# autowarefoundation/autoware_vision_pilot

Measured on NVIDIA H100. Metric: camera frames/sec @1080p multi-task, higher is better.
Workload: dtype f16

## Files before the change

autoware_vision_pilot_b200/csrc/conv_gemm.cu:

```cuda
#include "common.cuh"
#include "conv_gemm.cuh"
#include "ops_internal.h"
#include <cstdio>
#include <cstring>
#include <algorithm>

namespace vpb {

static constexpr int kMma = 256;
static constexpr int kEpilogue = 128;
static constexpr int kThreads = kMma + kEpilogue + 32;
static constexpr int kParts = kEpilogue / 128;
static constexpr int kMaxStages = 8;
static constexpr int kATileBytes = 128 * 128;
static constexpr int kMaxDynSmem = 227 * 1024 - 4096;
__host__ __device__ constexpr int acc_pitch(int bn) { return bn + 4; }
__host__ __device__ constexpr size_t acc_bytes(int bn) { return static_cast<size_t>(128) * acc_pitch(bn) * 4; }

__device__ __forceinline__ void acc_ld16(uint32_t t, uint32_t (&r)[16]) {
  const uint32_t a = t << 2;
#pragma unroll
  for (int i = 0; i < 4; ++i)
    asm volatile("ld.shared.v4.b32 {%0, %1, %2, %3}, [%4];"
                 : "=r"(r[4 * i]), "=r"(r[4 * i + 1]), "=r"(r[4 * i + 2]), "=r"(r[4 * i + 3])
                 : "r"(a + 16u * i)
                 : "memory");
}

struct EpiPix {
  bool ok;
  bool zero;
  uint32_t ooff;
  uint32_t roff;
  uint32_t fpix;
  uint32_t img;
};

template <class E, int NC, bool TILEK>
__device__ __forceinline__ void epilogue_chunks(const ConvKParams& p, uint32_t t_row, int n0,
                                                const float* sbias, int part, const EpiPix& px) {
  const bool split = TILEK && p.split;
  const int nchunks = p.BN >> 4;
  typename E::T* out = reinterpret_cast<typename E::T*>(p.out);
  const typename E::T* res = reinterpret_cast<const typename E::T*>(p.res);
  typename E::T* out_lo = reinterpret_cast<typename E::T*>(p.out_lo);
  const typename E::T* res_lo = reinterpret_cast<const typename E::T*>(p.res_lo);
  for (int chunk0 = part; chunk0 < nchunks; chunk0 += kParts * NC) {
    uint32_t rr[NC][16];
#pragma unroll
    for (int c = 0; c < NC; ++c) acc_ld16(t_row + (chunk0 + kParts * c) * 16, rr[c]);
    float v[NC][16];
#pragma unroll
    for (int c = 0; c < NC; ++c) {
      const float4* sb4 = reinterpret_cast<const float4*>(sbias + (chunk0 + kParts * c) * 16);
#pragma unroll
      for (int i = 0; i < 4; ++i) {
        const float4 b4 = sb4[i];
        const float2 lo = fadd2(make_float2(__uint_as_float(rr[c][4 * i]), __uint_as_float(rr[c][4 * i + 1])), make_float2(b4.x, b4.y));
        const float2 hi = fadd2(make_float2(__uint_as_float(rr[c][4 * i + 2]), __uint_as_float(rr[c][4 * i + 3])), make_float2(b4.z, b4.w));
        v[c][4 * i] = lo.x; v[c][4 * i + 1] = lo.y; v[c][4 * i + 2] = hi.x; v[c][4 * i + 3] = hi.y;
      }
    }
    if (p.act == ACT_GELU) {
#pragma unroll
      for (int c = 0; c < NC; ++c)
#pragma unroll
        for (int i = 0; i < 8; ++i) {
          const float2 g = act_gelu2(make_float2(v[c][2 * i], v[c][2 * i + 1]));
          v[c][2 * i] = g.x; v[c][2 * i + 1] = g.y;
        }
    } else if (p.act == ACT_SILU) {
#pragma unroll
      for (int c = 0; c < NC; ++c)
#pragma unroll
        for (int i = 0; i < 16; ++i) v[c][i] = act_silu(v[c][i]);
    } else if (p.act == ACT_SIGMOID) {
#pragma unroll
      for (int c = 0; c < NC; ++c)
#pragma unroll
        for (int i = 0; i < 16; ++i) v[c][i] = (n0 + (chunk0 + kParts * c) * 16 + i < p.Cout) ? act_sigmoid(v[c][i]) : 0.f;
    }
    if (p.mode == VPB_EPI_FINAL) {
      if (px.ok && chunk0 == 0) {
        const uint32_t plane = static_cast<uint32_t>(p.H * p.W);
        float* of = p.out_f32 + px.img * static_cast<uint32_t>(p.Cout) * plane;
#pragma unroll
        for (int i = 0; i < 16; ++i)
          if (i < p.Cout) of[i * plane + px.fpix] = v[0][i];
        if (p.out_cls) {
          uint8_t cls = 0;
          if (p.final_kind == VPB_FINAL_ARGMAX) {
            float best = v[0][0];
#pragma unroll
            for (int i = 1; i < 16; ++i)
              if (i < p.Cout && v[0][i] > best) { best = v[0][i]; cls = static_cast<uint8_t>(i); }
          } else if (p.final_kind == VPB_FINAL_THRESH) {
            cls = v[0][0] > 0.f ? 1 : 0;
          } else if (p.final_kind == VPB_FINAL_EGOLANES) {
            cls = (v[0][2] > 0.f) ? 2 : (v[0][1] > 0.f) ? 1 : (v[0][0] > 0.f) ? 0 : 255;
          }
          p.out_cls[px.img * plane + px.fpix] = cls;
        }
      }
    } else if (px.ok) {
      if (p.mode == VPB_EPI_ADD || p.mode == VPB_EPI_MULADD) {
        uint4 rv[NC][2];
        bool rok[NC][2];
#pragma unroll
        for (int c = 0; c < NC; ++c) {
          const int n = n0 + (chunk0 + kParts * c) * 16;
          const typename E::T* rp = res + (px.roff + n);
#pragma unroll
          for (int j = 0; j < 2; ++j) {
            rok[c][j] = (n + 8 * j < p.ldr) && (n + 8 * j < p.nlim);
            rv[c][j] = rok[c][j] ? *reinterpret_cast<const uint4*>(rp + 8 * j) : make_uint4(0, 0, 0, 0);
          }
        }
        uint4 rl[NC][2];
#pragma unroll
        for (int c = 0; c < NC; ++c)
#pragma unroll
          for (int j = 0; j < 2; ++j)
            rl[c][j] = (split && rok[c][j])
                           ? *reinterpret_cast<const uint4*>(res_lo + (px.roff + n0 + (chunk0 + kParts * c) * 16) + 8 * j)
                           : make_uint4(0, 0, 0, 0);
#pragma unroll
        for (int c = 0; c < NC; ++c)
#pragma unroll
          for (int j = 0; j < 2; ++j) {
            if (!rok[c][j]) continue;
            const uint32_t rw[4] = {rv[c][j].x, rv[c][j].y, rv[c][j].z, rv[c][j].w};
            const uint32_t rwl[4] = {rl[c][j].x, rl[c][j].y, rl[c][j].z, rl[c][j].w};
#pragma unroll
            for (int i = 0; i < 4; ++i) {
              float2 f = unpack2<E>(rw[i]);
              if (split) { const float2 fl = unpack2<E>(rwl[i]); f.x += fl.x; f.y += fl.y; }
              float& a = v[c][8 * j + 2 * i];
              float& b = v[c][8 * j + 2 * i + 1];
              if (p.mode == VPB_EPI_ADD) { a += f.x; b += f.y; }
              else { a = fmaf(a, f.x, f.x); b = fmaf(b, f.y, f.y); }
              if (TILEK && p.act2 == ACT_SILU) { a = act_silu(a); b = act_silu(b); }
            }
          }
      }
#pragma unroll
      for (int c = 0; c < NC; ++c) {
        const int n = n0 + (chunk0 + kParts * c) * 16;
        typename E::T* op = out + (px.ooff + n);
#pragma unroll
        for (int j = 0; j < 2; ++j) {
          if (n + 8 * j < p.nlim) {
            uint4 o;
            o.x = pack2<E>(v[c][8 * j + 0], v[c][8 * j + 1]);
            o.y = pack2<E>(v[c][8 * j + 2], v[c][8 * j + 3]);
            o.z = pack2<E>(v[c][8 * j + 4], v[c][8 * j + 5]);
// ... 290 lines not shown
      if (et < BN) {
        const int nn = n0 + et;
        s_bias[et] = (p.bias && nn < p.Cout) ? __ldg(p.bias + (p.upc ? 4 * p.Cout : 0) + nn) : 0.f;
      }
      named_bar_sync(1, kEpilogue);
      mbar_wait_quiet(smem_u32(&acc_full), acc_phase);

      if (p.upc) {
        const int pa = ph >> 1, pb = ph & 1;
        const int cy = (pa == 0 && h == 0) ? 0 : (pa == 1 && h == p.H - 1) ? 2 : 1;
        const int cx = (pb == 0 && w == 0) ? 0 : (pb == 1 && w == p.W - 1) ? 2 : 1;
        const int cls = cy * 3 + cx;
        const float* gb = cls != 4 ? p.bias + cls * p.Cout + n0 : nullptr;
        const int oh = 2 * h + pa, ow = 2 * w + pb;
        EpiPix px;
        px.ok = (h < p.H) && (w < p.W);
        px.zero = false;
        px.ooff = img * p.out_img + static_cast<uint32_t>((oh + p.out_pad) * (Wo + 2 * p.out_pad) + (ow + p.out_pad)) * p.ldo;
        px.roff = 0; px.fpix = 0; px.img = 0;
        if (p.act == ACT_GELU) epilogue_store_fast<E, ACT_GELU, false, true>(p, t_row, n0, s_bias, part, px, gb);
        else epilogue_store_fast<E, ACT_NONE, false, true>(p, t_row, n0, s_bias, part, px, gb);
      } else {
        const int oh = (p.phases > 1) ? 2 * h + (ph >> 1) : h;
        const int ow = (p.phases > 1) ? 2 * w + (ph & 1) : w;
        EpiPix px;
        px.ok = (h < p.H) && (w < p.W);
        px.zero = false;
        px.ooff = img * p.out_img + static_cast<uint32_t>((oh + p.out_pad) * (Wo + 2 * p.out_pad) + (ow + p.out_pad)) * p.ldo;
        px.roff = img * p.res_img + static_cast<uint32_t>((oh + p.res_pad) * (Wo + 2 * p.res_pad) + (ow + p.res_pad)) * p.ldr;
        px.fpix = static_cast<uint32_t>(h * p.W + w);
        px.img = static_cast<uint32_t>(img);
        epilogue_tile<E>(p, t_row, n0, s_bias, part, px);
      }
      mbar_arrive(smem_u32(&acc_empty));
      acc_phase ^= 1u;
    }
  }
}

__global__ void zero_border_kernel(uint4* out, int H, int W, int ldo, int nlim) {
  pdl_wait();
  out += (static_cast<size_t>(blockIdx.y) * (H + 2) * (W + 2) * ldo) >> 3;
  const int per = nlim >> 3, nb = 2 * (W + 2) + 2 * H;
  for (int i = blockIdx.x * blockDim.x + threadIdx.x; i < nb * per; i += gridDim.x * blockDim.x) {
    const int pix = i / per, v = i - pix * per;
    int y, x;
    if (pix < W + 2) { y = 0; x = pix; }
    else if (pix < 2 * (W + 2)) { y = H + 1; x = pix - (W + 2); }
    else { const int q = pix - 2 * (W + 2); y = 1 + (q >> 1); x = (q & 1) ? W + 1 : 0; }
    out[((static_cast<size_t>(y) * (W + 2) + x) * ldo >> 3) + v] = make_uint4(0, 0, 0, 0);
  }
}



typedef CUresult (*EncodeTiledFn)(CUtensorMap*, CUtensorMapDataType, cuuint32_t, void*,
                                  const cuuint64_t*, const cuuint64_t*, const cuuint32_t*,
                                  const cuuint32_t*, CUtensorMapInterleave, CUtensorMapSwizzle,
                                  CUtensorMapL2promotion, CUtensorMapFloatOOBfill);

static EncodeTiledFn get_encode_fn() {
  static EncodeTiledFn fn = nullptr;
  if (!fn) {
    void* p = nullptr;
    cudaDriverEntryPointQueryResult q;
    if (cudaGetDriverEntryPoint("cuTensorMapEncodeTiled", &p, cudaEnableDefault, &q) ==
            cudaSuccess &&
        q == cudaDriverEntryPointSuccess)
      fn = reinterpret_cast<EncodeTiledFn>(p);
  }
  return fn;
}

int device_sm_count() {
  int dev = 0, n = 0;
  cudaGetDevice(&dev);
  cudaDeviceGetAttribute(&n, cudaDevAttrMultiProcessorCount, dev);
  return n > 0 ? n : 132;
}

static int pick_bn(int Cout, int want) {
  if (want > 0) return want <= 16 ? 16 : want <= 32 ? 32 : want <= 64 ? 64 : 128;
  for (int bn : {128, 64, 32}) {
    if (Cout <= bn && (Cout > bn / 2 || bn == 32)) return bn;
    if (Cout > bn && (Cout + bn - 1) / bn * bn - Cout <= Cout / 4) return bn;
  }
  return 16;
}

int conv_plan_build(const vpb_conv_args* a, ConvPlan* plan) {
  if (!a || !plan) return VPB_ERR_ARG;
  if (a->Cin <= 0 || (a->Cin & 7) || (a->ldi & 7) || a->ldi < a->Cin) {
    vpb_set_error("conv: Cin=%d ldi=%d must be multiples of 8 (ldi >= Cin)", a->Cin, a->ldi);
    return VPB_ERR_ARG;
  }
  const int cstride = a->stride == 2 ? 2 : 1;
  if (a->stride != 0 && a->stride != 1 && a->stride != 2) { vpb_set_error("conv: stride %d unsupported", a->stride); return VPB_ERR_ARG; }
  if (cstride == 2 && (a->algo == VPB_ALGO_LINEAR || a->phases != 1 || a->in_pad || a->in2 || a->in_lo)) {
    vpb_set_error("conv: stride 2 needs the TILE algorithm on an unpadded input, phases = 1, no second input");
    return VPB_ERR_ARG;
  }
  if (a->ldw != 0 && (a->ldw < a->Cin || (a->ldw & 7) || a->algo == VPB_ALGO_LINEAR)) {
    vpb_set_error("conv: ldw=%d must be a multiple of 8 >= Cin (TILE algorithm)", a->ldw);
    return VPB_ERR_ARG;
  }
  if (a->act2 != ACT_NONE && a->act2 != ACT_SILU) { vpb_set_error("conv: act2 supports SiLU only"); return VPB_ERR_ARG; }
  const bool upc = a->taps == 4 && a->phases == 4;
  if (upc && (a->algo == VPB_ALGO_LINEAR || a->in_lo || a->mode != VPB_EPI_STORE || (a->act != ACT_NONE && a->act != ACT_GELU) ||
              !a->bias || (a->Cout & 15) || a->out_slice || cstride != 1 || a->ldw || (a->in2 && a->taps2 != 9))) {
    vpb_set_error("conv: upconv (taps=4, phases=4) needs the TILE algorithm, 16-bit mode, STORE, act NONE|GELU, bias[9][Cout], Cout%%16==0, taps2=9 with in2");
    return VPB_ERR_ARG;
  }
  if (!((a->taps == 9 && a->phases == 1) || (a->taps == 1 && (a->phases == 1 || a->phases == 4)) || upc)) {
    vpb_set_error("conv: unsupported taps=%d phases=%d", a->taps, a->phases);
    return VPB_ERR_ARG;
  }
  const bool lin = a->algo == VPB_ALGO_LINEAR;
  if (lin && (a->taps != 9 || !a->in_pad)) {
    vpb_set_error("conv: the linear-padded algorithm needs a 3x3 conv on a zero-bordered input");
    return VPB_ERR_ARG;
  }
  if (a->mode == VPB_EPI_FINAL) {
    if (a->Cout > 16 || !a->out_f32) {
      vpb_set_error("conv: FINAL mode needs Cout<=16 and out_f32");
      return VPB_ERR_ARG;
    }
  } else {
    if (!a->out || (a->ldo & 7) || a->ldo < a->Cout) {
      vpb_set_error("conv: bad out/ldo=%d (Cout=%d)", a->ldo, a->Cout);
      return VPB_ERR_ARG;
    }
    if ((a->mode == VPB_EPI_ADD || a->mode == VPB_EPI_MULADD) && (!a->res || (a->ldr & 7))) {
      vpb_set_error("conv: residual mode needs res with ldr%%8==0");
      return VPB_ERR_ARG;
    }
  }
  const bool split = a->in_lo != nullptr;
  if (split) {
    if (lin || !a->w_lo || (a->mode != VPB_EPI_FINAL && !a->out_lo) ||
        ((a->mode == VPB_EPI_ADD || a->mode == VPB_EPI_MULADD) && !a->res_lo) || (a->in2 && (!a->in2_lo || !a->w2_lo))) {
      vpb_set_error("conv: split-fp16 mode needs the TILE algorithm and the low halves of every tensor given (w_lo, out_lo, res_lo, in2_lo, w2_lo)");
      return VPB_ERR_ARG;
    }
  }
  if (a->in2) {
    if (lin || (a->taps != 1 && !upc) || !a->w2 || a->Cin2 <= 0 || (a->Cin2 & 7) || (a->ld2 & 7) || a->ld2 < a->Cin2) {
      vpb_set_error("conv: second input needs the TILE algorithm, taps=1, w2, Cin2/ld2 multiples of 8 (Cin2=%d ld2=%d)",
                    a->Cin2, a->ld2);
      return VPB_ERR_ARG;
    }
  }
  if (a->batch < 0) { vpb_set_error("conv: batch %d", a->batch); return VPB_ERR_ARG; }
  const int batch = a->batch > 0 ? a->batch : 1;
  if (a->w_img != 0) {
    const long ldw = a->ldw > 0 ? a->ldw : a->Cin;
    const char* why = a->algo == VPB_ALGO_LINEAR ? "the LINEAR algorithm has one weight operand"
                      : a->taps * a->phases != 1 ? "taps * phases must be 1"
                      : a->in2 ? "no second input"
                      : a->in_lo ? "no split-fp16 mode"
                      : (a->w_img & 7) ? "w_img must be a multiple of 8"
                      : a->w_img < ldw * a->Cout ? "w_img < ldw * Cout: the images' weight operands overlap"
                      : nullptr;
    if (why) { vpb_set_error("conv: per-image weights (w_img=%d): %s", a->w_img, why); return VPB_ERR_ARG; }
  }
  {
    const long ho = a->phases == 4 ? 2L * a->H + 2 : a->H + 2, wo = a->phases == 4 ? 2L * a->W + 2 : a->W + 2;
    if (ho * wo * std::max(a->ldo, a->ldr) * batch >= (1L << 31) || static_cast<long>(a->H) * a->W * 16 * batch >= (1L << 31)) {
      vpb_set_error("conv: tensor too large for 32-bit element offsets");
      return VPB_ERR_ARG;
    }
  }
  EncodeTiledFn enc = get_encode_fn();
  if (!enc) {
    vpb_set_error("conv: cuTensorMapEncodeTiled unavailable (no CUDA driver?)");
    return VPB_ERR_CUDA;
  }

  memset(plan, 0, sizeof(*plan));
  ConvKParams& p = plan->p;
  p.H = a->H; p.W = a->W; p.Cin = a->Cin; p.Cout = a->Cout;
  p.taps = a->taps; p.phases = a->phases;
  p.in_pad = a->in_pad ? 1 : 0; p.out_pad = a->out_pad ? 1 : 0; p.res_pad = a->res_pad ? 1 : 0;
  p.lin = (lin && a->out_pad && a->mode != VPB_EPI_FINAL) ? 1 : 0;
  p.split = split ? 1 : 0;
  p.w_img = a->w_img != 0 ? 1 : 0;
  p.stride = cstride; p.act2 = a->act2;
  p.nlim = a->out_slice ? std::min(a->ldo, (a->Cout + 7) / 8 * 8) : a->ldo;
  p.out_lo = a->out_lo; p.res_lo = a->res_lo;
  p.upc = upc ? 1 : 0;
  if (upc) {
    p.BN = 16;
    for (int bn : {128, 64, 32})
      if (a->Cout % bn == 0 && (a->bn <= 0 || bn <= a->bn)) { p.BN = bn; break; }
  } else {
    p.BN = pick_bn(a->Cout, a->bn);
  }
  p.tiles_n = (a->Cout + p.BN - 1) / p.BN;
  p.kchunks = (a->Cin + 63) / 64;
  p.Cin2 = a->in2 ? a->Cin2 : 0;
  p.kchunks2 = (p.Cin2 + 63) / 64;
  int best_tw = 128; long best_cost = -1;
  for (int tw = 128; tw >= 8; tw >>= 1) {
    const int th = 128 / tw;
    const long cost = static_cast<long>((a->H + th - 1) / th) * ((a->W + tw - 1) / tw);
    if (best_cost < 0 || cost < best_cost) { best_cost = cost; best_tw = tw; }
  }
  p.TW = best_tw; p.TH = 128 / best_tw;
  p.tw_shift = 0; while ((1 << p.tw_shift) < p.TW) ++p.tw_shift;
  p.tiles_h = (a->H + p.TH - 1) / p.TH;
  p.tiles_w = (a->W + p.TW - 1) / p.TW;
  p.tiles_img = p.tiles_h * p.tiles_w * p.tiles_n * p.phases;
  p.total_tiles = p.tiles_img * batch;
  p.mg_ti = fast_div_magic(p.tiles_img);
  {
    const long ho = a->phases == 4 ? 2L * a->H : a->H, wo = a->phases == 4 ? 2L * a->W : a->W;
    p.out_img = static_cast<uint32_t>((ho + 2 * p.out_pad) * (wo + 2 * p.out_pad) * a->ldo);
    p.res_img = static_cast<uint32_t>((ho + 2 * p.res_pad) * (wo + 2 * p.res_pad) * a->ldr);
  }
  const size_t stage_bytes = kATileBytes + static_cast<size_t>(p.BN) * 128;
  p.stages = static_cast<int>(std::min<size_t>(kMaxStages, (kMaxDynSmem - 1024 - acc_bytes(p.BN)) / stage_bytes));
// ... 101 lines not shown
}

template <class E, int BN>
static cudaError_t set_smem_attr() {
  return cudaFuncSetAttribute(conv_wgmma_kernel<E, BN>, cudaFuncAttributeMaxDynamicSharedMemorySize, kMaxDynSmem);
}

template <class E>
static cudaError_t launch_conv(const ConvPlan* plan, const ConvMaps& maps, cudaStream_t stream) {
  const dim3 g(plan->grid), b(kThreads);
  switch (plan->p.BN) {
    case 16: return launch_k(conv_wgmma_kernel<E, 16>, g, b, plan->smem_bytes, stream, maps, plan->p);
    case 32: return launch_k(conv_wgmma_kernel<E, 32>, g, b, plan->smem_bytes, stream, maps, plan->p);
    case 64: return launch_k(conv_wgmma_kernel<E, 64>, g, b, plan->smem_bytes, stream, maps, plan->p);
    default: return launch_k(conv_wgmma_kernel<E, 128>, g, b, plan->smem_bytes, stream, maps, plan->p);
  }
}

int conv_plan_launch(const ConvPlan* plan, cudaStream_t stream) {
  {
    std::lock_guard<std::mutex> g(init_mutex());
    bool* done = device_flag(kInitConv);
    if (!*done) {
      VPB_CUDA_OK((set_smem_attr<F16, 16>())); VPB_CUDA_OK((set_smem_attr<F16, 32>()));
      VPB_CUDA_OK((set_smem_attr<F16, 64>())); VPB_CUDA_OK((set_smem_attr<F16, 128>()));
      VPB_CUDA_OK((set_smem_attr<BF16, 16>())); VPB_CUDA_OK((set_smem_attr<BF16, 32>()));
      VPB_CUDA_OK((set_smem_attr<BF16, 64>())); VPB_CUDA_OK((set_smem_attr<BF16, 128>()));
      *done = true;
    }
  }
  ConvMaps maps;
  maps.A = plan->mapA; maps.B = plan->mapB; maps.A2 = plan->mapA2; maps.B2 = plan->mapB2;
  maps.Alo = plan->mapAlo; maps.Blo = plan->mapBlo; maps.A2lo = plan->mapA2lo; maps.B2lo = plan->mapB2lo;
  if (plan->dtype == VPB_BF16) VPB_CUDA_OK(launch_conv<BF16>(plan, maps, stream));
  else VPB_CUDA_OK(launch_conv<F16>(plan, maps, stream));
  if (plan->p.lin) {
    const ConvKParams& p = plan->p;
    const int n = (2 * (p.W + 2) + 2 * p.H) * (p.nlim >> 3);
    VPB_CUDA_OK(launch_k(zero_border_kernel, dim3(std::min((n + 255) / 256, 256), p.total_tiles / p.tiles_img), dim3(256), 0, stream,
                         static_cast<uint4*>(p.out), p.H, p.W, p.ldo, p.nlim));
  }
  return VPB_OK;
}

}


extern "C" int vpb_conv_gemm(const vpb_conv_args* a, void* stream) {
  vpb::ConvPlan plan;
  int rc = vpb::conv_plan_build(a, &plan);
  if (rc != VPB_OK) return rc;
  return vpb::conv_plan_launch(&plan, static_cast<cudaStream_t>(stream));
}
```

autoware_vision_pilot_b200/csrc/engine.cu:

```cuda
#include "common.cuh"
#include "conv_gemm.cuh"
#include "ops_internal.h"
#include "../../include/vp_b200.h"
#include "engine_internal.h"

#include <cmath>
#include <cstring>
#include <functional>
#include <map>
#include <memory>
#include <string>
#include <vector>

namespace vpb {

static uint64_t fnv1a(uint64_t h, const void* p, size_t n) {
  const uint8_t* b = static_cast<const uint8_t*>(p);
  for (size_t i = 0; i < n; ++i) { h ^= b[i]; h *= 1099511628211ull; }
  return h;
}
static uint64_t hash_prefix(const WeightMap& w, const std::string& pfx) {
  uint64_t h = 1469598103934665603ull;
  for (const auto& kv : w) {
    if (kv.first.compare(0, pfx.size(), pfx) != 0) continue;
// ... 351 lines not shown
    const int in_f = dims[i], out_f = dims[i + 1], a = acts[i];
    const float* xin = cur;
    e.add_op(tag + "mlp" + std::to_string(i), "linear_kernel", [=](cudaStream_t st) { return linear_x(xin, dw_, db, in_f, out_f, a, y, st, nb); },
             2.0 * in_f * out_f, 4.0 * in_f * out_f);
    cur = y;
  }
  const HostTensor *w3 = find_w_shaped(w, p + "context_layer_3.weight", {128, 1, 3, 3}), *b3 = find_w_shaped(w, p + "context_layer_3.bias", {128});
  if (!w3 || !b3) return VPB_ERR_IO;
  float *d_w3 = e.upload_f32(w3->f), *d_b3 = e.upload_f32(b3->f);
  Tens c4 = e.act_alloc(feat.H, feat.W, 128, 1);
  {
    const float* xin = cur; void* o = c4.p; void* o_lo = c4.lo; const int H = feat.H, W = feat.W;
    e.add_op(tag + "ctx3", "ctx_conv1_kernel", [=](cudaStream_t st) { return ctx_conv1_x(dt, xin, H, W, d_w3, d_b3, 128, o, o_lo, 1, st, VPB_ACT_GELU, nb); },
             2.0 * HW * 128 * 9, nb * 2.0 * (H + 2) * (W + 2) * 128);
  }
  Tens c5, c6;
  int rc = conv_layer(e, w, p + "context_layer_4", tag + "ctx4", c4, 9, ACT_GELU, VPB_EPI_STORE, &c5, nullptr);
  if (rc) return rc;
  rc = conv_layer(e, w, p + "context_layer_5", tag + "ctx5", c5, 9, ACT_GELU, VPB_EPI_STORE, &c6, nullptr);
  if (rc) return rc;
  *ctx = e.act_alloc(feat.H, feat.W, C, 1);
  return conv_layer(e, w, p + "context_layer_6", tag + "ctx6", c6, 9, ACT_GELU, VPB_EPI_MULADD, ctx, &feat);
}

static int build_neck(vp_engine& e, const WeightMap& w, const std::string& p, const std::string& tag,
                      const Tens& ctx, const vp_engine::EncOut& enc, Tens* neck) {
  Tens d = ctx, u;
  const int skip_src[3] = {3, 2, 1};
  for (int b = 0; b < 3; ++b) {
    Tens a, c;
    int rc;
    if (upconv_enabled(e)) {
      rc = upconv_layer(e, w, p, b, 2 * b, tag, d, &enc.f[skip_src[b]], &a);
      if (rc) return rc;
    } else {
      rc = up_skip(e, w, p, b, tag, d, &enc.f[skip_src[b]], &u);
      if (rc) return rc;
      rc = conv_layer(e, w, p + "decode_layer_" + std::to_string(2 * b), tag + "dec" + std::to_string(2 * b), u, 9, ACT_GELU, VPB_EPI_STORE, &a, nullptr);
      if (rc) return rc;
    }
    rc = conv_layer(e, w, p + "decode_layer_" + std::to_string(2 * b + 1), tag + "dec" + std::to_string(2 * b + 1), a, 9, ACT_GELU, VPB_EPI_STORE, &c, nullptr);
    if (rc) return rc;
    d = c;
  }
  *neck = d;
  return VPB_OK;
}

static int final_conv(vp_engine& e, const WeightMap& w, const std::string& key, const std::string& name,
                      const Tens& in, int final_kind, ModelOut& mo) {
  const HostTensor* wt = find_w_shaped(w, key + ".weight", {-1, in.C, 3, 3});
  const HostTensor* bt = wt ? find_w_shaped(w, key + ".bias", {wt->dims[0]}) : nullptr;
  if (!wt || !bt) return VPB_ERR_IO;
  const int Cout = wt->dims[0];
  void* dw_ = e.upload_16(pack_conv(*wt, nullptr));
  float* db = e.upload_f32(bt->f);
  mo.C = Cout; mo.H = in.H; mo.W = in.W;
  const size_t n = static_cast<size_t>(Cout) * in.H * in.W;
  const size_t nb = e.batch;
  mo.d_raw = static_cast<float*>(e.dalloc(n * 4 * nb, false));
  mo.has_cls = final_kind != VPB_FINAL_NONE;
  if (mo.has_cls) mo.d_cls = static_cast<uint8_t*>(e.dalloc(static_cast<size_t>(in.H) * in.W * nb, false));
  mo.h_raw = static_cast<float*>(e.halloc(n * 4 * nb));
  if (mo.has_cls) mo.h_cls = static_cast<uint8_t*>(e.halloc(static_cast<size_t>(in.H) * in.W * nb));
  if (!mo.h_raw || (mo.has_cls && !mo.h_cls)) return VPB_ERR_CUDA;
  return e.add_conv(name, in, Cout, 9, 1, dw_, db, ACT_NONE, VPB_EPI_FINAL, nullptr, nullptr, final_kind, mo.d_raw, mo.d_cls);
}

static int build_head(vp_engine& e, const WeightMap& w, const std::string& p, const std::string& tag, int kind,
                      const Tens& neck, const vp_engine::EncOut& enc, ModelOut& mo) {
  int rc;
  if (kind == VP_EGO_LANES) {
    Tens a, b;
    rc = conv_layer(e, w, p + "decode_layer_6", tag + "dec6", neck, 9, ACT_GELU, VPB_EPI_STORE, &a, nullptr); if (rc) return rc;
    rc = conv_layer(e, w, p + "decode_layer_7", tag + "dec7", a, 9, ACT_GELU, VPB_EPI_STORE, &b, nullptr); if (rc) return rc;
    return final_conv(e, w, p + "decode_layer_8", tag + "dec8", b, VPB_FINAL_EGOLANES, mo);
  }
  Tens u3, a, b, u4, c, d;
  if (upconv_enabled(e)) {
    rc = upconv_layer(e, w, p, 3, 6, tag, neck, &enc.f[0], &a); if (rc) return rc;
    rc = conv_layer(e, w, p + "decode_layer_7", tag + "dec7", a, 9, ACT_GELU, VPB_EPI_STORE, &b, nullptr); if (rc) return rc;
    rc = upconv_layer(e, w, p, 4, 8, tag, b, nullptr, &c); if (rc) return rc;
  } else {
    rc = up_skip(e, w, p, 3, tag, neck, &enc.f[0], &u3); if (rc) return rc;
    rc = conv_layer(e, w, p + "decode_layer_6", tag + "dec6", u3, 9, ACT_GELU, VPB_EPI_STORE, &a, nullptr); if (rc) return rc;
    rc = conv_layer(e, w, p + "decode_layer_7", tag + "dec7", a, 9, ACT_GELU, VPB_EPI_STORE, &b, nullptr); if (rc) return rc;
    rc = up_skip(e, w, p, 4, tag, b, nullptr, &u4); if (rc) return rc;
    rc = conv_layer(e, w, p + "decode_layer_8", tag + "dec8", u4, 9, ACT_GELU, VPB_EPI_STORE, &c, nullptr); if (rc) return rc;
  }
  rc = conv_layer(e, w, p + "decode_layer_9", tag + "dec9", c, 9, ACT_GELU, VPB_EPI_STORE, &d, nullptr); if (rc) return rc;
  e.tap(tag + "d9", d);
  const int fk = kind == VP_SCENE_SEG ? VPB_FINAL_ARGMAX : kind == VP_DOMAIN_SEG ? VPB_FINAL_THRESH : VPB_FINAL_NONE;
  return final_conv(e, w, p + "decode_layer_10", tag + "dec10", d, fk, mo);
}

static int build_model(vp_engine& e, int idx, int kind, const WeightMap& w) {
  const Prefixes pf = prefixes_for(kind);
  const std::string tag = std::to_string(idx) + "/";
  const uint64_t h_enc = hash_prefix(w, pf.enc);
  e.cur_lane = idx;
  int dep = -1;
  vp_engine::EncOut enc;
  auto ie = e.enc_cache.find(h_enc);
  if (ie != e.enc_cache.end()) { enc = ie->second; ++e.shared_encoders; dep = e.enc_last_op[h_enc]; }
  else {
    int rc = build_encoder(e, w, pf.enc, tag, enc);
    if (rc) return rc;
    e.enc_cache[h_enc] = enc;
    e.enc_last_op[h_enc] = static_cast<int>(e.ops.size()) - 1;
  }
  for (int i = 0; i < 5; ++i) e.tap(tag + "f" + std::to_string(i), enc.f[i]);
  uint64_t h_trunk = h_enc;
  { const uint64_t a = hash_prefix(w, pf.ctx), b = hash_prefix(w, pf.neck); h_trunk = fnv1a(fnv1a(h_trunk, &a, 8), &b, 8); }
  Tens neck;
  auto it = e.trunk_cache.find(h_trunk);
  if (it != e.trunk_cache.end()) { neck = it->second; ++e.shared_trunks; dep = e.trunk_last_op[h_trunk]; }
  else {
    Tens feat = enc.f[4];
    if (kind == VP_EGO_LANES) {
// ... 392 lines not shown
```

autoware_vision_pilot_b200/csrc/engine_common.cu:

```cuda
#include "common.cuh"
#include "conv_gemm.cuh"
#include "engine_internal.h"

#include <cstdio>
#include <cstdlib>
#include <cstring>

namespace vpb {

int load_vpw(const char* path, WeightMap& out) {
  FILE* fp = fopen(path, "rb");
  if (!fp) { vpb_set_error("cannot open weight file '%s'", path); return VPB_ERR_IO; }
  auto fail = [&](const char* why) { fclose(fp); vpb_set_error("%s: %s", path, why); return VPB_ERR_IO; };
  if (fseek(fp, 0, SEEK_END) != 0) return fail("cannot seek");
  const long file_size = ftell(fp);
  rewind(fp);
  char magic[4]; uint32_t n = 0;
  if (fread(magic, 1, 4, fp) != 4 || memcmp(magic, "VPW1", 4) != 0) return fail("not a VPW1 file");
  if (fread(&n, 4, 1, fp) != 1 || n > 100000) return fail("bad tensor count");
  for (uint32_t i = 0; i < n; ++i) {
    uint32_t nl = 0, dt = 0, nd = 0; uint64_t nb = 0;
    if (fread(&nl, 4, 1, fp) != 1 || nl > 4096) return fail("bad name length");
    std::string name(nl, '\0');
    if (fread(&name[0], 1, nl, fp) != nl) return fail("truncated name");
// ... 5 lines not shown
    bool dims_ok = true;
    for (int d : t.dims) {
      if (d < 0 || (d > 0 && ne > (static_cast<size_t>(1) << 31) / static_cast<size_t>(d))) { dims_ok = false; break; }
      ne *= static_cast<size_t>(d);
    }
    if (!dims_ok) return fail("tensor dims out of range");
    if (dt == 0) {
      if (nb != ne * 4) return fail("f32 size mismatch");
      t.f.resize(ne);
      if (ne && fread(t.f.data(), 4, ne, fp) != ne) return fail("truncated data");
    } else {
      const long here = ftell(fp);
      if (here < 0 || nb > static_cast<uint64_t>(file_size - here) || fseek(fp, static_cast<long>(nb), SEEK_CUR) != 0)
        return fail("truncated data");
    }
    out[name] = std::move(t);
  }
  fclose(fp);
  return VPB_OK;
}

const HostTensor* find_w(const WeightMap& w, const std::string& key) {
  auto it = w.find(key);
  if (it == w.end()) { vpb_set_error("weight '%s' missing from checkpoint", key.c_str()); return nullptr; }
  return &it->second;
}

const HostTensor* find_w_shaped(const WeightMap& w, const std::string& key, std::initializer_list<int> dims) {
  const HostTensor* t = find_w(w, key);
  if (!t) return nullptr;
  bool ok = t->dims.size() == dims.size() && t->f.size() == t->numel();
  if (ok) { size_t i = 0; for (int d : dims) { if (d >= 0 && t->dims[i] != d) ok = false; ++i; } }
  if (!ok) {
    std::string got, want;
    for (int d : t->dims) got += std::to_string(d) + ",";
    for (int d : dims) want += (d < 0 ? std::string("*") : std::to_string(d)) + ",";
    vpb_set_error("weight '%s' has shape [%s] but this architecture needs [%s]", key.c_str(), got.c_str(), want.c_str());
    return nullptr;
  }
  return t;
}

std::vector<float> pack_conv(const HostTensor& t, const std::vector<float>* scale) {
  const int Cout = t.dims[0], Cin = t.dims[1], k = t.dims[2];
  std::vector<float> o(t.f.size());
  for (int co = 0; co < Cout; ++co)
    for (int ci = 0; ci < Cin; ++ci)
      for (int tt = 0; tt < k * k; ++tt)
        o[(static_cast<size_t>(tt) * Cout + co) * Cin + ci] =
            t.f[(static_cast<size_t>(co) * Cin + ci) * k * k + tt] * (scale ? (*scale)[co] : 1.0f);
  return o;
}

int FrameGraph::run(cudaStream_t st, const PreprocessPlan& pre, int dtype, int h_, int w_, int stride_,
                    const FrameSrcs& src_, const std::function<int(cudaStream_t)>& launch,
                    const std::function<int(cudaGraphExec_t, cudaGraphNode_t)>& repoint) {
  const bool same_geometry = exec && h == h_ && w == w_ && stride == stride_;
  if (same_geometry && src != src_ && pre_node) {
    const int rc = repoint(exec, pre_node);
    if (rc) return rc;
    src = src_;
  }
  if (!same_geometry || src != src_) {
    invalidate();
    pre_node = nullptr;
    int rc = launch(st);
    if (rc) return rc;
    VPB_CUDA_OK(cudaStreamSynchronize(st));
    cudaGraph_t g = nullptr;
    VPB_CUDA_OK(cudaStreamBeginCapture(st, cudaStreamCaptureModeThreadLocal));
    rc = launch(st);
    cudaError_t ce = cudaStreamEndCapture(st, &g);
    if (rc) { if (g) cudaGraphDestroy(g); return rc; }
    if (ce != cudaSuccess) { vpb_set_error("graph capture failed: %s", cudaGetErrorString(ce)); return VPB_ERR_CUDA; }
    size_t nn = 0;
    cudaGraphGetNodes(g, nullptr, &nn);
    std::vector<cudaGraphNode_t> nodes(nn);
    cudaGraphGetNodes(g, nodes.data(), &nn);
    for (size_t i = 0; i < nn; ++i) {
      cudaGraphNodeType ty;
      if (cudaGraphNodeGetType(nodes[i], &ty) != cudaSuccess || ty != cudaGraphNodeTypeKernel) continue;
      cudaKernelNodeParams kp{};
      if (cudaGraphKernelNodeGetParams(nodes[i], &kp) == cudaSuccess && pre.owns_kernel(kp.func, dtype)) {
        pre_node = nodes[i];
        break;
      }
    }
    ce = cudaGraphInstantiate(&exec, g, 0);
    if (graph) cudaGraphDestroy(graph);
    graph = g;
    if (ce != cudaSuccess) { vpb_set_error("graph instantiate failed: %s", cudaGetErrorString(ce)); return VPB_ERR_CUDA; }
    h = h_; w = w_; stride = stride_; src = src_;
  }
  VPB_CUDA_OK(cudaGraphLaunch(exec, st));
  return VPB_OK;
}

void FrameGraph::invalidate() {
  if (exec) { cudaGraphExecDestroy(exec); exec = nullptr; }
}

void FrameGraph::release() {
  invalidate();
  if (graph) { cudaGraphDestroy(graph); graph = nullptr; }
}

// ... 188 lines not shown
```

autoware_vision_pilot_b200/csrc/ops_internal.h:

```cpp
#pragma once
#include <cuda_runtime.h>
#include <stdint.h>
#include <vector>
#include <mutex>
#include "../../include/vp_b200_ops.h"

namespace vpb {

static constexpr int kNetH = 320, kNetW = 640;
static constexpr int kGapReplicas = 8;
static constexpr int kMaxBatch = 8;

void resize_tables_host(int mode, int in_size, int out_size, std::vector<int>& bounds,
                        std::vector<int>& coeffs, int& ksize);

struct PreprocessPlan {
  int h = 0, w = 0, mode = -1;
  int OH = kNetH, OW = kNetW;
  int xks = 0, yks = 0;
  int rows_cap = 0, patch_w_cap = 0;
  int TY = 20, pitch = 0, xt = 16;
  int device = -1;
  void* out_lo = nullptr;
  int out_pitch = 0, out_x0 = 0, out_y0 = 0, out_c = 4, out_rows = 0;
  size_t smem_bytes = 0;
  int* d_tables = nullptr;
  size_t off_xb = 0, off_xk = 0, off_yb = 0, off_yk = 0;
  int configure(int in_h, int in_w, int mode);
  int launch(const uint8_t* const* srcs, int batch, int stride, int convention, int dtype, void* out, uint8_t* out_u8,
             cudaStream_t stream) const;
  bool owns_kernel(const void* func, int dtype) const;
  int update_graph_node(cudaGraphExec_t exec, cudaGraphNode_t node, const uint8_t* const* srcs, int batch, int stride,
                        int convention, int dtype, void* out, uint8_t* out_u8) const;
  ~PreprocessPlan();
};

struct DwGeom {
  int Ho, Wo, G, PPB, threads, pix_per_block, nblocks;
};
DwGeom dw_geometry(int H, int W, int C, int k, int stride);

int stem_conv_x(int dtype, const void* in, const void* in_lo, int H, int W, const float* w, const float* bias,
                void* out, void* out_lo, cudaStream_t st, int batch = 1);
int depthwise_x(int dtype, const void* in, const void* in_lo, int H, int W, int C, int k, int stride, const float* w,
                const float* bias, void* out, void* out_lo, long long* gap_acc, cudaStream_t st,
                int act = VPB_ACT_SILU , int batch = 1);
int se_scale_x(int dtype, const long long* gap_acc, int HW, int C, int sq, const float* w1, const float* b1,
               const float* w2, const float* b2, void* act, void* act_lo, float* scale_out, cudaStream_t st, int batch = 1);
int gap_x(int dtype, const void* in, const void* in_lo, int HW, int C, int ld, float* out, cudaStream_t st, int batch = 1);
int linear_x(const float* x, const float* w, const float* b, int in_f, int out_f, int act, float* y, cudaStream_t st,
             int batch);
int ctx_conv1_x(int dtype, const float* in, int H, int W, const float* w, const float* b, int Cout, void* out,
                void* out_lo, int out_pad, cudaStream_t st, int act = VPB_ACT_GELU , int batch = 1);
int fuse_pool_x(int dtype, const void* f0, const void* f1, const void* f2, const void* f3, const void* f4,
                const size_t lo_off[5], int H4, int W4, void* out, void* out_lo, cudaStream_t st, int batch = 1);

enum InitSlot { kInitConv = 0, kInitPreprocess = 1, kInitVizTable = 2, kInitSlots = 4 };
std::mutex& init_mutex();
bool* device_flag(InitSlot slot);

}
```

include/vp_b200_ops.h:

```cpp
#ifndef VP_B200_OPS_H_
#define VP_B200_OPS_H_
#include <stddef.h>
#include <stdint.h>

#ifdef __cplusplus
extern "C" {
#endif

enum { VPB_OK = 0, VPB_ERR_ARG = -1, VPB_ERR_CUDA = -2, VPB_ERR_STATE = -3, VPB_ERR_IO = -4 };
enum { VPB_F16 = 0, VPB_BF16 = 1 };
enum { VPB_ACT_NONE = 0, VPB_ACT_GELU = 1, VPB_ACT_SILU = 2, VPB_ACT_SIGMOID = 3, VPB_ACT_SILU2 = 4  };
enum {
  VPB_EPI_STORE = 0,
  VPB_EPI_ADD = 1,
  VPB_EPI_MULADD = 2,
  VPB_EPI_FINAL = 3
};
enum {
  VPB_FINAL_NONE = 0,
  VPB_FINAL_ARGMAX = 1,
  VPB_FINAL_THRESH = 2,
  VPB_FINAL_EGOLANES = 3
};

enum { VPB_ALGO_TILE = 0, VPB_ALGO_LINEAR = 1 };

const char* vpb_last_error(void);
void vpb_set_error(const char* fmt, ...);

typedef struct {
  int dtype;
  int H, W, Cin, ldi;
  int Cout, taps, phases;
  int act, mode, final_kind;
  const void* in;
  const void* w;
  const float* bias;
  void* out;
  int ldo;
  const void* res;
  int ldr;
  float* out_f32;
  uint8_t* out_cls;
  int bn;
  int in_pad, out_pad, res_pad;
  int algo;
  int dbg_ms;
  int dbg_gb;
  int dbg_base_offset;
  const void* in2;
  const void* w2;
  int Cin2, ld2, in2_pad;
  int dbg_pair;
  int dbg_splitk;
  unsigned long long* dbg_trace;
  int stride, in_h, in_w;
  int ldw;
  int act2;
  int out_slice;
  const void* in_lo;
  const void* w_lo;
  void* out_lo;
  const void* res_lo;
  const void* in2_lo;
  const void* w2_lo;
  int taps2;
  int batch;
  int w_img;
} vpb_conv_args;
int vpb_conv_gemm(const vpb_conv_args* a, void* stream);
int vpb_upconv_compose(const float* w3, const float* b3, const float* wt, const float* bt, const float* ws,
                       const float* bs, int Cout, int Cmid, int Cin, int C2, float* wf, float* w2f, float* bias9,
                       void* stream);
int vpb_f32_to_16(int dtype, const float* src, void* dst, long long n, void* stream);

enum { VPB_RESIZE_NONE = 0, VPB_RESIZE_PIL_BICUBIC = 1, VPB_RESIZE_CV_LINEAR = 2,
       VPB_RESIZE_PIL_BILINEAR = 3  };
enum { VPB_CONV_RGB = 0, VPB_CONV_BGR_NOSWAP = 1, VPB_CONV_BGR_SWAP = 2,
       VPB_CONV_RGB_UNIT = 3  };
int vpb_preprocess(const uint8_t* src_dev, int h, int w, int stride, int resize_mode, int convention,
                   int dtype, void* out_dev, uint8_t* out_u8_dev, void* stream);
int vpb_resize_tables_host(int mode, int in_size, int out_size, int* bounds, int* coeffs,
                           int coeffs_cap, int* ksize);

int vpb_stem_conv(int dtype, const void* in, int H, int W, const float* w, const float* bias,
                  void* out, void* stream);
int vpb_depthwise(int dtype, const void* in, int H, int W, int C, int k, int stride, const float* w,
                  const float* bias, void* out, long long* gap_acc, void* stream);
int vpb_se_scale(int dtype, const long long* gap_acc, int HW, int C, int sq, const float* w1,
                 const float* b1, const float* w2, const float* b2, void* act, float* scale_out, void* stream);

int vpb_gap(int dtype, const void* in, int HW, int C, int ld, float* out, void* stream);
int vpb_linear(const float* x, const float* w, const float* b, int in_f, int out_f, int act, float* y,
               void* stream);
int vpb_ctx_conv1(int dtype, const float* in, int H, int W, const float* w, const float* b, int Cout,
                  void* out, int out_pad, void* stream);
int vpb_fuse_pool_concat(int dtype, const void* f0, const void* f1, const void* f2, const void* f3,
                         const void* f4, int H4, int W4, void* out, void* stream);

int vpb_stem_conv_ex(int dtype, const void* in, const void* in_lo, int H, int W, const float* w, const float* bias,
                     void* out, void* out_lo, int batch, void* stream);
int vpb_depthwise_ex(int dtype, const void* in, const void* in_lo, int H, int W, int C, int k, int stride,
                     const float* w, const float* bias, void* out, void* out_lo, long long* gap_acc, int act, int batch,
                     void* stream);
int vpb_se_scale_ex(int dtype, const long long* gap_acc, int HW, int C, int sq, const float* w1, const float* b1,
                    const float* w2, const float* b2, void* act, void* act_lo, float* scale_out, int batch, void* stream);
int vpb_gap_ex(int dtype, const void* in, const void* in_lo, int HW, int C, int ld, float* out, int batch, void* stream);
int vpb_linear_ex(const float* x, const float* w, const float* b, int in_f, int out_f, int act, float* y, int batch,
                  void* stream);
int vpb_ctx_conv1_ex(int dtype, const float* in, int H, int W, const float* w, const float* b, int Cout, void* out,
                     void* out_lo, int out_pad, int act, int batch, void* stream);
int vpb_fuse_pool_concat_ex(int dtype, const void* f0, const void* f1, const void* f2, const void* f3, const void* f4,
                            const void* f0_lo, const void* f1_lo, const void* f2_lo, const void* f3_lo,
                            const void* f4_lo, int H4, int W4, void* out, void* out_lo, int batch, void* stream);

int vpb_mask255(const float* raw, int channels, int rows, int cols, uint8_t* out, void* stream);
int vpb_egolanes_ids(const float* raw, int channels, int rows, int cols, uint8_t* out, void* stream);
int vpb_lane_masks(const float* raw, int n, float threshold, float* out, void* stream);
int vpb_resize_nearest_u8(const uint8_t* src, int sh, int sw, uint8_t* dst, int dh, int dw, void* stream);
int vpb_resize_linear_f32(const float* src, int sh, int sw, float* dst, int dh, int dw, void* stream);
enum { VPB_VIZ_SCENE = 0, VPB_VIZ_DOMAIN = 1, VPB_VIZ_EGOLANES = 2 };
int vpb_visualize_mask(const uint8_t* mask, int mh, int mw, int viz_type, const uint8_t* frame_bgr, int h,
                       int w, int stride, uint8_t* out, int out_stride, void* stream);
// ... 46 lines not shown
```

Measured before the change: 342.4.

## Split final 3x3 head conv into per-tap 1x1 GEMM plus tap-sum kernel

The final 3x3 output conv with tiny Cout is rewritten as a 1x1 conv producing 9*Cout per-tap partial maps in fp32, followed by a new kernel that sums the shifted taps, adds bias and computes the class map. The FINAL epilogue now handles multiple 16-channel chunks so Cout up to 32 works. The aim is to avoid the inefficient 3x3 implicit-GEMM path for a head with very few output channels. The cost is an extra kernel launch and writing and re-reading a 9*Cout fp32 intermediate at full resolution.

```diff
diff --git a/autoware_vision_pilot_b200/csrc/conv_gemm.cu b/autoware_vision_pilot_b200/csrc/conv_gemm.cu
--- a/autoware_vision_pilot_b200/csrc/conv_gemm.cu
+++ b/autoware_vision_pilot_b200/csrc/conv_gemm.cu
@@ -25,6 +25,21 @@
                  : "=r"(r[4 * i]), "=r"(r[4 * i + 1]), "=r"(r[4 * i + 2]), "=r"(r[4 * i + 3])
                  : "r"(a + 16u * i)
                  : "memory");
+}
+
+__device__ __forceinline__ uint8_t final_class(int kind, const float (&v)[16], int Cout) {
+  uint8_t cls = 0;
+  if (kind == VPB_FINAL_ARGMAX) {
+    float best = v[0];
+#pragma unroll
+    for (int i = 1; i < 16; ++i)
+      if (i < Cout && v[i] > best) { best = v[i]; cls = static_cast<uint8_t>(i); }
+  } else if (kind == VPB_FINAL_THRESH) {
+    cls = v[0] > 0.f ? 1 : 0;
+  } else if (kind == VPB_FINAL_EGOLANES) {
+    cls = (v[2] > 0.f) ? 2 : (v[1] > 0.f) ? 1 : (v[0] > 0.f) ? 0 : 255;
+  }
+  return cls;
 }
 
 struct EpiPix {
@@ -81,26 +96,14 @@
         for (int i = 0; i < 16; ++i) v[c][i] = (n0 + (chunk0 + kParts * c) * 16 + i < p.Cout) ? act_sigmoid(v[c][i]) : 0.f;
     }
     if (p.mode == VPB_EPI_FINAL) {
-      if (px.ok && chunk0 == 0) {
+      if (px.ok) {
         const uint32_t plane = static_cast<uint32_t>(p.H * p.W);
-        float* of = p.out_f32 + px.img * static_cast<uint32_t>(p.Cout) * plane;
+        const int c0 = n0 + chunk0 * 16;
+        float* of = p.out_f32 + (px.img * static_cast<uint32_t>(p.Cout) + c0) * plane;
 #pragma unroll
         for (int i = 0; i < 16; ++i)
-          if (i < p.Cout) of[i * plane + px.fpix] = v[0][i];
-        if (p.out_cls) {
-          uint8_t cls = 0;
-          if (p.final_kind == VPB_FINAL_ARGMAX) {
-            float best = v[0][0];
-#pragma unroll
-            for (int i = 1; i < 16; ++i)
-              if (i < p.Cout && v[0][i] > best) { best = v[0][i]; cls = static_cast<uint8_t>(i); }
-          } else if (p.final_kind == VPB_FINAL_THRESH) {
-            cls = v[0][0] > 0.f ? 1 : 0;
-          } else if (p.final_kind == VPB_FINAL_EGOLANES) {
-            cls = (v[0][2] > 0.f) ? 2 : (v[0][1] > 0.f) ? 1 : (v[0][0] > 0.f) ? 0 : 255;
-          }
-          p.out_cls[px.img * plane + px.fpix] = cls;
-        }
+          if (c0 + i < p.Cout) of[i * plane + px.fpix] = v[0][i];
+        if (p.out_cls && c0 == 0) p.out_cls[px.img * plane + px.fpix] = final_class(p.final_kind, v[0], p.Cout);
       }
     } else if (px.ok) {
       if (p.mode == VPB_EPI_ADD || p.mode == VPB_EPI_MULADD) {
@@ -497,6 +500,57 @@
   }
 }
 
+static constexpr int kTapsumMaxC = 3;
+__global__ void __launch_bounds__(256) final_tapsum_kernel(const float* __restrict__ P, const float* __restrict__ bias,
+                                                           int Cout, int H, int W, int kind, float* __restrict__ out,
+                                                           uint8_t* __restrict__ cls) {
+  pdl_launch_dependents();
+  pdl_wait();
+  const int HW = H * W;
+  const int pix = blockIdx.x * blockDim.x + threadIdx.x;
+  if (pix >= HW) return;
+  const int y = pix / W, x = pix - y * W;
+  const float* pi = P + static_cast<size_t>(blockIdx.y) * 9 * Cout * HW;
+  int off[9];
+  uint32_t inside = 0;
+#pragma unroll
+  for (int t = 0; t < 9; ++t) {
+    const int yy = y + t / 3 - 1, xx = x + t % 3 - 1;
+    off[t] = t * Cout * HW + yy * W + xx;
+    if (yy >= 0 && yy < H && xx >= 0 && xx < W) inside |= 1u << t;
+  }
+  float p[9][kTapsumMaxC];
+#pragma unroll
+  for (int t = 0; t < 9; ++t)
+#pragma unroll
+    for (int o = 0; o < kTapsumMaxC; ++o)
+      p[t][o] = (o < Cout && (inside & (1u << t))) ? __ldg(pi + (off[t] + o * HW)) : 0.f;
+  float v[16] = {};
+#pragma unroll
+  for (int o = 0; o < kTapsumMaxC; ++o) {
+    if (o >= Cout) continue;
+#pragma unroll
+    for (int t = 0; t < 9; ++t)
+      if (inside & (1u << t)) v[o] += p[t][o];
+    if (bias) v[o] += __ldg(bias + o);
+    out[(static_cast<size_t>(blockIdx.y) * Cout + o) * HW + pix] = v[o];
+  }
+  if (cls) cls[static_cast<size_t>(blockIdx.y) * HW + pix] = final_class(kind, v, Cout);
+}
+
+int final_tapsum_x(const float* P, const float* bias, int Cout, int H, int W, int final_kind, float* out, uint8_t* cls,
+                   cudaStream_t st, int batch) {
+  if (!P || !out || Cout < 1 || Cout > kTapsumMaxC || H < 1 || W < 1 || batch < 1 || batch > kMaxBatch ||
+      final_kind < VPB_FINAL_NONE || final_kind > VPB_FINAL_EGOLANES) {
+    vpb_set_error("final_tapsum: bad arguments (Cout %d must be 1..%d, batch %d 1..%d, H %d, W %d, final_kind %d)", Cout,
+                  kTapsumMaxC, batch, kMaxBatch, H, W, final_kind);
+    return VPB_ERR_ARG;
+  }
+  if (static_cast<long>(H) * W * 9 * kTapsumMaxC >= (1L << 31)) { vpb_set_error("final_tapsum: image too large"); return VPB_ERR_ARG; }
+  const dim3 grid((H * W + 255) / 256, batch);
+  VPB_CUDA_OK(launch_k(final_tapsum_kernel, grid, dim3(256), 0, st, P, bias, Cout, H, W, final_kind, out, cls));
+  return VPB_OK;
+}
 
 
 typedef CUresult (*EncodeTiledFn)(CUtensorMap*, CUtensorMapDataType, cuuint32_t, void*,
@@ -566,8 +620,8 @@
     return VPB_ERR_ARG;
   }
   if (a->mode == VPB_EPI_FINAL) {
-    if (a->Cout > 16 || !a->out_f32) {
-      vpb_set_error("conv: FINAL mode needs Cout<=16 and out_f32");
+    if (a->Cout > 32 || (a->out_cls && a->Cout > 16) || !a->out_f32) {
+      vpb_set_error("conv: FINAL mode needs Cout<=32 (<=16 with a class map) and out_f32");
       return VPB_ERR_ARG;
     }
   } else {
@@ -610,7 +664,7 @@
   }
   {
     const long ho = a->phases == 4 ? 2L * a->H + 2 : a->H + 2, wo = a->phases == 4 ? 2L * a->W + 2 : a->W + 2;
-    if (ho * wo * std::max(a->ldo, a->ldr) * batch >= (1L << 31) || static_cast<long>(a->H) * a->W * 16 * batch >= (1L << 31)) {
+    if (ho * wo * std::max(a->ldo, a->ldr) * batch >= (1L << 31) || static_cast<long>(a->H) * a->W * (a->mode == VPB_EPI_FINAL ? std::max(a->Cout, 16) : 16) * batch >= (1L << 31)) {
       vpb_set_error("conv: tensor too large for 32-bit element offsets");
       return VPB_ERR_ARG;
     }
@@ -818,3 +872,8 @@
   if (rc != VPB_OK) return rc;
   return vpb::conv_plan_launch(&plan, static_cast<cudaStream_t>(stream));
 }
+
+extern "C" int vpb_final_tapsum(const float* P, const float* bias, int Cout, int H, int W, int final_kind, float* out,
+                                uint8_t* cls, int batch, void* stream) {
+  return vpb::final_tapsum_x(P, bias, Cout, H, W, final_kind, out, cls, static_cast<cudaStream_t>(stream), batch);
+}
diff --git a/autoware_vision_pilot_b200/csrc/engine.cu b/autoware_vision_pilot_b200/csrc/engine.cu
--- a/autoware_vision_pilot_b200/csrc/engine.cu
+++ b/autoware_vision_pilot_b200/csrc/engine.cu
@@ -427,19 +427,26 @@
   const HostTensor* wt = find_w_shaped(w, key + ".weight", {-1, in.C, 3, 3});
   const HostTensor* bt = wt ? find_w_shaped(w, key + ".bias", {wt->dims[0]}) : nullptr;
   if (!wt || !bt) return VPB_ERR_IO;
-  const int Cout = wt->dims[0];
+  const int Cout = wt->dims[0], H = in.H, W = in.W, nb = e.batch;
   void* dw_ = e.upload_16(pack_conv(*wt, nullptr));
   float* db = e.upload_f32(bt->f);
-  mo.C = Cout; mo.H = in.H; mo.W = in.W;
-  const size_t n = static_cast<size_t>(Cout) * in.H * in.W;
-  const size_t nb = e.batch;
-  mo.d_raw = static_cast<float*>(e.dalloc(n * 4 * nb, false));
+  mo.C = Cout; mo.H = H; mo.W = W;
+  const size_t plane = static_cast<size_t>(H) * W;
+  mo.d_raw = static_cast<float*>(e.dalloc(plane * Cout * 4 * nb, false));
   mo.has_cls = final_kind != VPB_FINAL_NONE;
-  if (mo.has_cls) mo.d_cls = static_cast<uint8_t*>(e.dalloc(static_cast<size_t>(in.H) * in.W * nb, false));
-  mo.h_raw = static_cast<float*>(e.halloc(n * 4 * nb));
-  if (mo.has_cls) mo.h_cls = static_cast<uint8_t*>(e.halloc(static_cast<size_t>(in.H) * in.W * nb));
+  if (mo.has_cls) mo.d_cls = static_cast<uint8_t*>(e.dalloc(plane * nb, false));
+  mo.h_raw = static_cast<float*>(e.halloc(plane * Cout * 4 * nb));
+  if (mo.has_cls) mo.h_cls = static_cast<uint8_t*>(e.halloc(plane * nb));
   if (!mo.h_raw || (mo.has_cls && !mo.h_cls)) return VPB_ERR_CUDA;
-  return e.add_conv(name, in, Cout, 9, 1, dw_, db, ACT_NONE, VPB_EPI_FINAL, nullptr, nullptr, final_kind, mo.d_raw, mo.d_cls);
+  float* d_taps = static_cast<float*>(e.dalloc(plane * 9 * Cout * 4 * nb, false));
+  int rc = e.add_conv(name + "taps", in, 9 * Cout, 1, 1, dw_, nullptr, ACT_NONE, VPB_EPI_FINAL, nullptr, nullptr,
+                      VPB_FINAL_NONE, d_taps);
+  if (rc) return rc;
+  float* raw = mo.d_raw; uint8_t* cls = mo.d_cls;
+  e.add_op(name + "sum", "final_tapsum_kernel",
+           [=](cudaStream_t st) { return final_tapsum_x(d_taps, db, Cout, H, W, final_kind, raw, cls, st, nb); },
+           0.0, nb * (4.0 * 10 * Cout * plane + (cls ? plane : 0)));
+  return VPB_OK;
 }
 
 static int build_head(vp_engine& e, const WeightMap& w, const std::string& p, const std::string& tag, int kind,
diff --git a/autoware_vision_pilot_b200/csrc/engine_common.cu b/autoware_vision_pilot_b200/csrc/engine_common.cu
--- a/autoware_vision_pilot_b200/csrc/engine_common.cu
+++ b/autoware_vision_pilot_b200/csrc/engine_common.cu
@@ -81,6 +81,20 @@
   return o;
 }
 
+}
+
+extern "C" int vpb_final_conv_weights_host(const float* w, int Cout, int Cin, float* out) {
+  if (!w || !out || Cout < 1 || Cin < 1) { vpb_set_error("final_conv_weights: bad arguments"); return VPB_ERR_ARG; }
+  vpb::HostTensor t;
+  t.dims = {Cout, Cin, 3, 3};
+  t.f.assign(w, w + t.numel());
+  const std::vector<float> o = vpb::pack_conv(t, nullptr);
+  memcpy(out, o.data(), o.size() * sizeof(float));
+  return VPB_OK;
+}
+
+namespace vpb {
+
 int FrameGraph::run(cudaStream_t st, const PreprocessPlan& pre, int dtype, int h_, int w_, int stride_,
                     const FrameSrcs& src_, const std::function<int(cudaStream_t)>& launch,
                     const std::function<int(cudaGraphExec_t, cudaGraphNode_t)>& repoint) {
diff --git a/autoware_vision_pilot_b200/csrc/ops_internal.h b/autoware_vision_pilot_b200/csrc/ops_internal.h
--- a/autoware_vision_pilot_b200/csrc/ops_internal.h
+++ b/autoware_vision_pilot_b200/csrc/ops_internal.h
@@ -54,6 +54,8 @@
                 void* out_lo, int out_pad, cudaStream_t st, int act = VPB_ACT_GELU , int batch = 1);
 int fuse_pool_x(int dtype, const void* f0, const void* f1, const void* f2, const void* f3, const void* f4,
                 const size_t lo_off[5], int H4, int W4, void* out, void* out_lo, cudaStream_t st, int batch = 1);
+int final_tapsum_x(const float* P, const float* bias, int Cout, int H, int W, int final_kind, float* out, uint8_t* cls,
+                   cudaStream_t st, int batch = 1);
 
 enum InitSlot { kInitConv = 0, kInitPreprocess = 1, kInitVizTable = 2, kInitSlots = 4 };
 std::mutex& init_mutex();
diff --git a/include/vp_b200_ops.h b/include/vp_b200_ops.h
--- a/include/vp_b200_ops.h
+++ b/include/vp_b200_ops.h
@@ -69,6 +69,9 @@
   int w_img;
 } vpb_conv_args;
 int vpb_conv_gemm(const vpb_conv_args* a, void* stream);
+int vpb_final_tapsum(const float* P, const float* bias, int Cout, int H, int W, int final_kind, float* out,
+                     uint8_t* cls, int batch, void* stream);
+int vpb_final_conv_weights_host(const float* w, int Cout, int Cin, float* out);
 int vpb_upconv_compose(const float* w3, const float* b3, const float* wt, const float* bt, const float* ws,
                        const float* bs, int Cout, int Cmid, int Cin, int C2, float* wf, float* w2f, float* bias9,
                        void* stream);
```

New measurement: 355.9 (median of 6 runs). +3.9%, better.
